# yaokeepmoving/distributed_tensorflow

Measured on AMD Instinct MI355X. Metric: images/sec (whole node) ResNet-50 bf16 at 1/2/4/8 MI355X; scaling efficiency, higher is better.
Workload: dtype bf16; 1 GPU; model=ResNet-50 v1.5, image_size=224, hiprio=True, hipgraph=True, graph_streams=2, global_batch=1024, per_gpu_batch=1024, parallelism=dp1, optimizer=SGD, allreduce_dtype=f32, zero1=False, forced_collective=False

## Files before the change

csrc/kernels/c3wgrad.hip:

```cpp
#include "gemm_core.h"

namespace dtf {
namespace {

constexpr int C3_SLOT = 72 * 128;
constexpr int C3_NS = 8;
constexpr int C3_DY = 64 * 128;
constexpr int C3_NB = 4;
constexpr int C3_JUNK = 8192;
constexpr int C3_SMEM = C3_NS * C3_SLOT + C3_NB * C3_DY + C3_JUNK;
constexpr int C3_OUT = 64 * 9 * 64;

struct C3Args {
  const bf16_t* X;
  const bf16_t* dY;
  float* ws;
  int H, W;
  long rows;
  int rpb;
};

__device__ __forceinline__ v8bf c3_tr_pair(uint32_t a0, uint32_t a1) {
  v4s r0, r1;
  asm volatile("ds_read_b64_tr_b16 %0, %1" : "=v"(r0) : "v"(a0));
// ... 92 lines not shown
  for (int it = 0; it < n_mine; ++it) {
    if (it + 2 < n_mine) asm volatile("s_waitcnt vmcnt(16)" ::: "memory");
    else if (it + 1 < n_mine) asm volatile("s_waitcnt vmcnt(8)" ::: "memory");
    else asm volatile("s_waitcnt vmcnt(0)" ::: "memory");
    asm volatile("s_waitcnt lgkmcnt(0)\n\ts_barrier" ::: "memory");
    if (it + C3_NB - 1 < n_mine) issue(it + C3_NB - 1, in, ih);
    next(in, ih);
    const char* img = dyi + (it % C3_NB) * C3_DY;
    const char* xr[3];
#pragma unroll
    for (int ta = 0; ta < 3; ++ta) xr[ta] = xs + ((n * VH + h + ta) & (C3_NS - 1)) * C3_SLOT;
    v8bf fx[2][9], fy[2][4];
    auto load = [&](int ks, v8bf(&x)[9], v8bf(&y)[4]) {
#pragma unroll
      for (int ta = 0; ta < 3; ++ta)
#pragma unroll
        for (int tb = 0; tb < 3; ++tb) x[ta * 3 + tb] = c3_frag(xr[ta], 16 * wave, tb, ks, lane);
#pragma unroll
      for (int j = 0; j < 4; ++j) y[j] = c3_frag(img, 16 * j, 0, ks, lane);
    };
    load(0, fx[0], fy[0]);
#pragma unroll
    for (int ks = 0; ks < 2; ++ks) {
      asm volatile("s_waitcnt lgkmcnt(0)" ::: "memory");
#pragma unroll
      for (int u = 0; u < 9; ++u) asm volatile("" : "+v"(fx[ks][u]));
#pragma unroll
      for (int j = 0; j < 4; ++j) asm volatile("" : "+v"(fy[ks][j]));
      if (ks == 0) load(1, fx[1], fy[1]);
#pragma unroll
      for (int u = 0; u < 9; ++u)
#pragma unroll
        for (int j = 0; j < 4; ++j)
          acc[u][j] = __builtin_amdgcn_mfma_f32_16x16x32_bf16(fx[ks][u], fy[ks][j], acc[u][j], 0, 0, 0);
    }
    next(n, h);
  }

  float* slab = a.ws + (long)blockIdx.x * C3_OUT;
#pragma unroll
  for (int u = 0; u < 9; ++u)
#pragma unroll
    for (int j = 0; j < 4; ++j) {
      const int k = 16 * j + (lane & 15), c = 16 * wave + 4 * (lane >> 4);
      *reinterpret_cast<float4*>(slab + ((long)k * 9 + u) * 64 + c) =
          make_float4(acc[u][j][0], acc[u][j][1], acc[u][j][2], acc[u][j][3]);
    }
}

}

int c3_wgrad_try(const void* X, const void* dY, float* dW, int N, int H, int W, int accumulate, float* ws,
                 long ws_elems, hipStream_t st) {
  if (((uintptr_t)X & 15) || ((uintptr_t)dY & 15) || !ws || N < 1 || H < 1 || W < 1 || W > 64) return -1;
  if ((long)N * (H + 2) >= (1l << 31)) return -1;
  C3Args a{};
  a.X = (const bf16_t*)X; a.dY = (const bf16_t*)dY; a.ws = ws;
  a.H = H; a.W = W;
  a.rows = (long)N * H;
  int grid = 256;
  while (grid > 8 && (long)grid * C3_OUT > ws_elems) grid /= 2;
  if ((long)grid * C3_OUT > ws_elems) return -1;
  a.rpb = (int)((a.rows + grid - 1) / grid);
  grid = (int)((a.rows + a.rpb - 1) / a.rpb);
  hipLaunchKernelGGL(c3_wgrad_kernel, dim3(grid), dim3(256), 0, st, a);
  if (hipGetLastError() != hipSuccess) return -1;
  dtf_sum_rows(ws, C3_OUT, grid, C3_OUT, dW, accumulate, st);
  return (int)hipGetLastError();
}

}
```

csrc/kernels/gemm.hip:

```cpp
#include <cstdlib>

#include "gemm_core.h"

__global__ void __launch_bounds__(256) dtf_group_rows_kernel(float* __restrict__ rows, long stride, int nrows,
                                                             int sg, long W, float* __restrict__ out,
                                                             int accumulate) {
  const long i = (long)blockIdx.x * blockDim.x + threadIdx.x;
  if (i >= W) return;
  const int r0 = blockIdx.y * sg;
  const int r1 = min(nrows, r0 + sg);
  float a8[8] = {0, 0, 0, 0, 0, 0, 0, 0};
  int r = r0;
  for (; r + 8 <= r1; r += 8) {
#pragma unroll
    for (int u = 0; u < 8; ++u) a8[u] += rows[(long)(r + u) * stride + i];
  }
  for (; r < r1; ++r) a8[0] += rows[(long)r * stride + i];
  const float acc = ((a8[0] + a8[1]) + (a8[2] + a8[3])) + ((a8[4] + a8[5]) + (a8[6] + a8[7]));
  if (out) out[i] = accumulate ? out[i] + acc : acc;
  else rows[(long)r0 * stride + i] = acc;
}

__global__ void __launch_bounds__(256) dtf_group_rows4_kernel(float* __restrict__ rows, long stride, int nrows,
                                                              int sg, long W4, float* __restrict__ out,
// ... 598 lines not shown
    long t = i;
    const int kc = (int)(t % k8); t /= k8;
    const int jw = (int)(t % nkw); t /= nkw;
    const int j = (int)(t % nkh);
    const int c = (int)(t / nkh);
    const long so = (((long)c * R + rh + sh * j) * S + rw + sw * jw) * K + kc * 8;
    *reinterpret_cast<uint4*>(dst + i * 8) = *reinterpret_cast<const uint4*>(src + so);
  }
}

static int conv_dgrad_impl(const void* dY, const void* Wcrsk, void* dX, int N, int H, int W, int C, int K, int R,
                           int S, int P, int Q, int sh, int sw, int ph, int pw, int dh, int dw, int out_f32,
                           float beta, int tile, void* ws, long ws_bf16, const void* bnx, const void* bnmask,
                           const float* bnmean, float* bnpart, int* bnrows, const void* betamask,
                           const void* bsrc2, void* stream, const void* bnrx = nullptr, const void* bnrw = nullptr);

namespace dtf {
int pwconv_dgrad_try(const void* dY, const void* Wck, void* dX, float beta, const void* betamask, const void* bnx,
                     const void* bnmask, const float* bnmean, float* part, long M, int Kc, int N, const void* bsrc2,
                     int H, int W, hipStream_t st, const void* bnrx, const void* bnrw);
}
static int g_pw_dgrad = -1;
static bool pwdgrad_enabled() {
  if (g_pw_dgrad < 0) {
    const char* e = getenv("DTF_PW_DGRAD");
    g_pw_dgrad = !(e && e[0] == '0');
  }
  return g_pw_dgrad != 0;
}
DTF_API int dtf_set_pw_dgrad(int on) {
  g_pw_dgrad = on ? 1 : 0;
  return 0;
}
namespace dtf {
int pw_wgrad_try(const void* X, const void* dY, float* dW, long P, int C, int K, int accumulate, float* ws,
                 long ws_elems, hipStream_t st, bool split_out);
}
namespace dtf {
int c3_wgrad_try(const void* X, const void* dY, float* dW, int N, int H, int W, int accumulate, float* ws,
                 long ws_elems, hipStream_t st);
}
static int g_c3_wgrad = -1;
static bool c3wgrad_enabled() {
  if (g_c3_wgrad < 0) {
    const char* e = getenv("DTF_C3_WGRAD");
    g_c3_wgrad = !(e && e[0] == '0');
  }
  return g_c3_wgrad != 0;
}
DTF_API int dtf_set_c3_wgrad(int on) {
  g_c3_wgrad = on ? 1 : 0;
  return 0;
}
static int g_pw_wgrad = -1;
static bool pwwgrad_enabled() {
  if (g_pw_wgrad < 0) {
    const char* e = getenv("DTF_PW_WGRAD");
    g_pw_wgrad = e ? atoi(e) : 1;
  }
  return g_pw_wgrad != 0;
}
DTF_API int dtf_set_pw_wgrad(int on) {
  g_pw_wgrad = on;
  return 0;
}

DTF_API int dtf_conv_dgrad(const void* dY, const void* Wcrsk, void* dX, int N, int H, int W, int C, int K, int R,
                           int S, int P, int Q, int sh, int sw, int ph, int pw, int dh, int dw, int out_f32,
                           float beta, int tile, void* ws, long ws_bf16, const void* bnx, const void* bnmask,
                           const float* bnmean, float* bnpart, int* bnrows, const void* betamask,
                           void* stream) {
  return conv_dgrad_impl(dY, Wcrsk, dX, N, H, W, C, K, R, S, P, Q, sh, sw, ph, pw, dh, dw, out_f32, beta, tile, ws,
                         ws_bf16, bnx, bnmask, bnmean, bnpart, bnrows, betamask, nullptr, stream);
}

DTF_API int dtf_conv_dgrad_x(const void* dY, const void* Wcrsk, void* dX, int N, int H, int W, int C, int K, int R,
                             int S, int P, int Q, int sh, int sw, int ph, int pw, int dh, int dw, float beta, void* ws,
                             long ws_bf16, const void* bnx, const void* bnmask, const float* bnmean, float* bnpart,
                             int* bnrows, const void* betamask, const void* bsrc2, const void* bnrx, const void* bnrw,
                             void* stream) {
  if (bsrc2) {
    if ((H & 1) || (W & 1) || R != 1 || S != 1 || sh != 1 || sw != 1 || ph != 0 || pw != 0) return -11;
    return conv_dgrad_impl(dY, Wcrsk, dX, N, H, W, C, K, 1, 1, H, W, 1, 1, 0, 0, 1, 1, 0, 1.f, -1, ws, ws_bf16, bnx,
                           bnmask, bnmean, bnpart, bnrows, nullptr, bsrc2, stream, bnrx, bnrw);
  }
  return conv_dgrad_impl(dY, Wcrsk, dX, N, H, W, C, K, R, S, P, Q, sh, sw, ph, pw, dh, dw, 0, beta, -1, ws, ws_bf16,
                         bnx, bnmask, bnmean, bnpart, bnrows, betamask, nullptr, stream, bnrx, bnrw);
}

DTF_API int dtf_conv_dgrad_addsub2(const void* dY, const void* Wcrsk, void* dX, const void* bsrc2, int N, int H, int W,
                                   int C, int K, int tile, void* ws, long ws_bf16, const void* bnx,
                                   const void* bnmask, const float* bnmean, float* bnpart, int* bnrows,
                                   void* stream) {
  if ((H & 1) || (W & 1) || !bsrc2) return -11;
  return conv_dgrad_impl(dY, Wcrsk, dX, N, H, W, C, K, 1, 1, H, W, 1, 1, 0, 0, 1, 1, 0, 1.f, tile, ws, ws_bf16, bnx,
                         bnmask, bnmean, bnpart, bnrows, nullptr, bsrc2, stream);
}

static int conv_dgrad_impl(const void* dY, const void* Wcrsk, void* dX, int N, int H, int W, int C, int K, int R,
                           int S, int P, int Q, int sh, int sw, int ph, int pw, int dh, int dw, int out_f32,
                           float beta, int tile, void* ws, long ws_bf16, const void* bnx, const void* bnmask,
                           const float* bnmean, float* bnpart, int* bnrows, const void* betamask,
                           const void* bsrc2, void* stream, const void* bnrx, const void* bnrw) {
  if ((C & 3) || (K & 7)) return -1;
  if (bnrx && (bnx || !bnrw || !bnpart || !bnmean || !bnrows)) return -9;
  if (bnx && (out_f32 || (C & 7) || !bnpart || !bnmean || !bnrows)) return -9;
// ... 84 lines not shown
      a.lda = K; a.ldb = (long)nkh * nkw * K; a.ldc = C;
      a.batch = 1; a.splitk = 1; a.kchunk = (a.K + BK - 1) / BK * BK;
      a.alpha = 1.f; a.beta = beta; a.act = 0; a.out_f32 = out_f32;
      a.crm = 1;
      a.dRm1 = make_fastdiv((uint32_t)(Hs * Ws)); a.dRm2 = make_fastdiv((uint32_t)Ws);
      a.rmH = H; a.rmW = W; a.rmsh = sh; a.rmsw = sw; a.rmh0 = h0; a.rmw0 = w0;
      bn_args(a);
      const bool pointwise = nkh == 1 && nkw == 1 && ch == 0 && cw == 0 && Hs == P && Ws == Q;
      const int am = pointwise ? OP_KCONTIG
                     : tap_uniform(K, nkh * nkw, (long)N * P * Q * K) ? OP_DGRAD_T : OP_DGRAD;
      int t = tile;
      if (t >= 0 && try_conv256(a, am, OP_KCONTIG, t, st)) {
      } else {
        dispatch(a, am, OP_KCONTIG, t < 0 ? pick_glds_tile(a, am, OP_KCONTIG) : t, st);
      }
      prow += a.tiles_m;
    }
  }
  if (bnrows) *bnrows = bnx ? prow : 0;
  return (int)hipGetLastError();
}

DTF_API int dtf_conv_wgrad(const void* X, const void* dY, float* dW, int N, int H, int W, int C, int K, int R,
                           int S, int P, int Q, int sh, int sw, int ph, int pw, int dh, int dw, int accumulate,
                           int splitk, int tile, float* ws, long ws_elems, void* stream) {
  if ((C & 7) || (K & 7)) return -1;
  const int splitk_req = splitk;
  if (tile < 0 && C == 16 && R == 4 && S == 4 && K == 64) tile = 3;
  hipStream_t st = (hipStream_t)stream;
  GemmArgs a{};
  a.g = make_geom(N, H, W, C, K, R, S, P, Q, sh, sw, ph, pw, dh, dw);
  a.g_rowrep = rowrep(a.g.R, a.g.S);
  a.A = (const bf16_t*)dY; a.B = (const bf16_t*)X;
  a.M = K; a.N = R * S * C; a.K = N * P * Q;
  a.lda = K; a.ldb = C; a.ldc = (long)R * S * C;
  a.batch = 1;
  a.alpha = 1.f; a.beta = 0.f; a.act = 0; a.out_f32 = 1;
  const long mn = (long)a.M * a.N;
  if (splitk <= 0) splitk = choose_splitk(a.M, a.N, a.K, 128, 128, 1);
  if (ws == nullptr || ws_elems < mn * 2) splitk = 1;
  else if ((long)splitk * mn > ws_elems) splitk = (int)(ws_elems / mn);
  if (splitk < 1) splitk = 1;
  a.splitk = splitk;
  a.kchunk = ((a.K + splitk - 1) / splitk + BK - 1) / BK * BK;
  bool pointwise = R == 1 && S == 1 && sh == 1 && sw == 1 && ph == 0 && pw == 0;
  if (pointwise && tile < 0 && splitk_req <= 0 && pwwgrad_enabled() &&
      pw_wgrad_try(X, dY, dW, (long)N * H * W, C, K, accumulate, ws, ws_elems, st, g_pw_wgrad == 2) == 0)
    return 0;
  if (tile < 0 && splitk_req <= 0 && C == 64 && K == 64 && R == 3 && S == 3 && sh == 1 && sw == 1 && ph == 1 &&
      pw == 1 && dh == 1 && dw == 1 && P == H && Q == W && c3wgrad_enabled() &&
      c3_wgrad_try(X, dY, dW, N, H, W, accumulate, ws, ws_elems, st) == 0)
    return 0;
  const bool small = (long)N * H * W * C * 2 < (1l << 31) && (long)N * P * Q * K * 2 < (1l << 31);
  const bool use_glds = small && (tile >= 7 || (tile < 0 && R * S > 1));
  const bool rowmap = small && (use_glds || !pointwise);
  constexpr bool swap_on = true;
  constexpr bool c256w = false;
  const bool c256_forced = tile >= 11 && tile <= 14;
  if (small && ws != nullptr && (c256_forced || (tile < 0 && c256w && conv256_on())) &&
      (pointwise || (C % 8 == 0 && (dh == 1 && dw == 1)))) {
    GemmArgs b = a;
    b.A = (const bf16_t*)X; b.B = (const bf16_t*)dY;
    b.M = R * S * C; b.N = K;
    b.lda = C; b.ldb = K; b.ldc = K;
    const int cfg = c256_forced ? tile - 11 : (K <= 64 ? 2 : K >= 256 ? 1 : 0);
    const int bn = cfg == 1 ? 256 : cfg == 2 ? 64 : 128;
    const long mnT = (long)b.M * b.N;
    const long tiles = (long)cdiv(b.M, 256) * cdiv(b.N, bn);
    long sk = std::max<long>(1, (512 + tiles - 1) / tiles);
    sk = std::min<long>(sk, std::max<long>(1, (long)b.K / 1024));
    if ((sk + 1) * mnT > ws_elems) sk = ws_elems / mnT - 1;
    if (sk >= 1) {
      b.splitk = (int)sk;
      b.kchunk = (int)(((b.K + sk - 1) / sk + BK - 1) / BK * BK);
      b.C = ws;
      b.slab = mnT;
      b.beta = 0.f;
      b.atomic_out = 0;
      if (conv256_try(b, pointwise ? OP_KOUTER : OP_WGRADX_R, OP_KOUTER_R, cfg, st, true) == 0) {
        float* dwt = ws + (long)b.splitk * mnT;
        dtf_sum_rows(ws, mnT, b.splitk, mnT, dwt, 0, st);
        hipLaunchKernelGGL(transpose_acc_kernel, dim3(cdiv(b.N, 32), cdiv(b.M, 32)), dim3(256), 0, st, dwt, dW,
                           b.M, b.N, accumulate);
        return (int)hipGetLastError();
      }
    }
  }
  if (c256_forced) tile = -1;
  if (pointwise && tile < 0 && ws != nullptr && K >= 128 && C >= 128 && (long)K * C >= 4 * 256 * 128) {
    int bn = 0;
    const int s = plan_w4_split_long(a.M, a.N, a.K, 1, bn);
    if (bn && s >= 1 && (s == 1 || (long)s * mn <= ws_elems)) {
      GemmArgs b = a;
      b.splitk = s;
      b.kchunk = ((b.K + s - 1) / s + BK - 1) / BK * BK;
      if (s > 1) {
        b.C = ws;
        b.slab = mn;
        b.beta = 0.f;
      } else {
        b.C = dW;
        b.beta = accumulate ? 1.f : 0.f;
      }
      if (tile256_try(b, OP_KOUTER, OP_KOUTER, st, bn) == 0) {
        if (s > 1) {
          count_launch(LC_SPLITK);
          dtf_sum_rows(ws, mn, s, mn, dW, accumulate, st);
        }
        return (int)hipGetLastError();
      }
    }
  }
  if (swap_on && use_glds && tile < 0 && K <= 64 && R * S > 1 && ws != nullptr) {
    GemmArgs b = a;
    b.A = (const bf16_t*)X; b.B = (const bf16_t*)dY;
    b.M = R * S * C; b.N = K;
    b.lda = C; b.ldb = K; b.ldc = K;
    const long mnT = (long)b.M * b.N;
    int sk = choose_splitk(b.M, b.N, b.K, 128, 64, 1);
    if ((long)(sk + 1) * mnT > ws_elems) sk = (int)(ws_elems / mnT) - 1;
    if (sk >= 1) {
      b.splitk = sk;
      b.kchunk = ((b.K + sk - 1) / sk + BK - 1) / BK * BK;
      b.C = ws;
      b.slab = mnT;
      b.beta = 0.f;
      dispatch(b, OP_WGRADX_R, OP_KOUTER_R, 8, st);
      float* dwt = ws + (long)sk * mnT;
      dtf_sum_rows(ws, mnT, sk, mnT, dwt, 0, st);
      hipLaunchKernelGGL(transpose_acc_kernel, dim3(cdiv(b.N, 32), cdiv(b.M, 32)), dim3(256), 0, st, dwt, dW, b.M,
                         b.N, accumulate);
      return (int)hipGetLastError();
    }
  }
  if (tile < 0 && use_glds) tile = 7;
  if (tile < 0) {
    if (a.M <= 64) tile = pointwise && a.N >= 256 ? 4 : 3;
    else if (R * S > 1) tile = 0;
  }
  auto run = [&]() {
    dispatch(a, rowmap ? OP_KOUTER_R : OP_KOUTER, rowmap ? OP_WGRADX_R : pointwise ? OP_KOUTER : OP_WGRADX, tile, st);
  };
  if (splitk == 1) {
    a.C = dW;
    a.beta = accumulate ? 1.f : 0.f;
    run();
    return (int)hipGetLastError();
  }
  a.C = ws;
  a.slab = mn;
  run();
  dtf_sum_rows(ws, mn, splitk, mn, dW, accumulate, st);
  return (int)hipGetLastError();
}
```

csrc/kernels/gemm_core.h:

```cpp
#pragma once
#include "common.h"
#include <algorithm>
#include <type_traits>

namespace dtf {

enum OpMode : int {
  OP_KCONTIG = 0,
  OP_KOUTER = 1,
  OP_IM2COL = 2,
  OP_DGRAD = 3,
  OP_WGRADX = 4,
  OP_IM2COL_T = 5,
  OP_DGRAD_T = 6,
  OP_KOUTER_R = 7,
  OP_WGRADX_R = 8,
};

struct ConvGeom {
  int N, H, W, C;
  int Kout, R, S;
  int P, Q;
  int sh, sw, ph, pw, dh, dw;
  FastDiv dPQ, dQ, dHW, dW, dC, dS, dK;
};

struct GemmArgs {
  const bf16_t* A;
  const bf16_t* B;
  void* C;
  bf16_t* aux;
  const float* bias;
  const float* scales;
  float* stats;
  long lda, ldb, ldc;
  long sA, sB, sC;
  int M, N, K;
  int batch, splitk, kchunk;
  int tiles_m, tiles_n;
  float alpha, beta;
  int act;
  int out_f32;
  int atomic_out;
  long slab;
  ConvGeom g;
  uint64_t g_rowrep;
  const bf16_t* bnx;
  const uint8_t* bnmask;
  const float* bnmean;
  const uint8_t* betamask;
  const bf16_t* dact_src;
  int dact;
  float* zero_slot;
  const bf16_t* bsrc;
  FastDiv dBhw, dBw;
  int bH2, bW2;
  int crm;
  FastDiv dRm1, dRm2;
  int rmH, rmW, rmsh, rmsw, rmh0, rmw0;
  uint8_t* q8;
  uint8_t* q8T;
  float* q8col;
  const float* q8scale;
  float* q8amax;
  const float* q8amax_prev;
  float* q8used;
  float* q8used2;
  int q8fmt;
  int no_c;
  int aux_nt;
  float* rowsum;
};

__device__ __forceinline__ uint32_t q8pack4(int fmt, float a0, float a1, float a2, float a3) {
  int r;
  if (fmt) {
    r = __builtin_amdgcn_cvt_pk_bf8_f32(a0, a1, 0, false);
    r = __builtin_amdgcn_cvt_pk_bf8_f32(a2, a3, r, true);
  } else {
    r = __builtin_amdgcn_cvt_pk_fp8_f32(a0, a1, 0, false);
    r = __builtin_amdgcn_cvt_pk_fp8_f32(a2, a3, r, true);
  }
  return (uint32_t)r;
}

__device__ __forceinline__ long out_row(const GemmArgs& a, int m) {
  if (!a.crm) return m;
  uint32_t n, hw, hh, ww;
  fdivmod((uint32_t)m, a.dRm1, n, hw);
  fdivmod(hw, a.dRm2, hh, ww);
  return ((long)n * a.rmH + (long)(a.rmsh * (int)hh + a.rmh0)) * a.rmW + (a.rmsw * (int)ww + a.rmw0);
}

constexpr int BK = 64;
constexpr int NT = 256;

__device__ __forceinline__ const bf16_t* beta_src(const GemmArgs& a, long m, int n, const bf16_t* cp) {
  if (!a.bsrc) return cp;
  uint32_t nn, hw, h, w;
  fdivmod((uint32_t)m, a.dBhw, nn, hw);
  fdivmod(hw, a.dBw, h, w);
  if ((h | w) & 1u) return nullptr;
  return a.bsrc + (((long)nn * a.bH2 + (h >> 1)) * a.bW2 + (w >> 1)) * a.ldc + n;
}

__device__ __forceinline__ void stat_acc(const GemmArgs& a, long mrow, int n, const float (&v)[4], float (&cs)[4],
                                         float (&cq)[4]) {
  if (a.bnx) {
    const long e = mrow * a.ldc + n;
    const uint2 xr = *reinterpret_cast<const uint2*>(a.bnx + e);
    const float x[4] = {__uint_as_float(xr.x << 16), __uint_as_float(xr.x & 0xffff0000u),
                        __uint_as_float(xr.y << 16), __uint_as_float(xr.y & 0xffff0000u)};
    const uint32_t bits = a.bnmask ? ((uint32_t)a.bnmask[e >> 3] >> (e & 4)) : 0xFu;
    const float4 mu = *reinterpret_cast<const float4*>(a.bnmean + n);
    const float m4[4] = {mu.x, mu.y, mu.z, mu.w};
#pragma unroll
    for (int r = 0; r < 4; ++r) {
      const float dz = ((bits >> r) & 1u) ? v[r] : 0.f;
      cs[r] += dz;
      cq[r] = fmaf(dz, x[r] - m4[r], cq[r]);
    }
  } else {
#pragma unroll
    for (int r = 0; r < 4; ++r) { cs[r] += v[r]; cq[r] = fmaf(v[r], v[r], cq[r]); }
// ... 976 lines not shown
```

csrc/kernels/gemm_w4.h:

```cpp
#pragma once
#include <type_traits>

#include "gemm_core.h"

namespace dtf {
namespace {

constexpr int W4_THREADS = 256;
constexpr int W4_A = 256 * BK * 2;

__device__ __forceinline__ void w4_barrier() {
  __builtin_amdgcn_sched_barrier(0);
  asm volatile("" ::: "memory");
  __builtin_amdgcn_s_barrier();
  asm volatile("" ::: "memory");
  __builtin_amdgcn_sched_barrier(0);
}

__device__ __forceinline__ void w4_mfma_drain() {
  asm volatile("s_nop 7\n\ts_nop 7\n\ts_nop 7" ::: "memory");
}

__device__ __forceinline__ void w4_lgkm0() {
  __builtin_amdgcn_sched_barrier(0);
// ... 64 lines not shown
    dS = g.dS;
    if constexpr (MODE == OP_IM2COL_T) {
      dCh = g.dC;
      tsh = g.dh * g.W * g.C * 2;
      tsw = g.dw * g.C * 2;
      rsrc = __builtin_amdgcn_make_buffer_rsrc((void*)p, (short)0, (int)((long)g.N * g.H * g.W * g.C * 2), 0x00020000);
    } else {
      dCh = g.dK;
      tsh = -(g.dh * g.Q * g.Kout * 2);
      tsw = -(g.dw * g.Kout * 2);
      rsrc = __builtin_amdgcn_make_buffer_rsrc((void*)p, (short)0, (int)((long)g.N * g.P * g.Q * g.Kout * 2),
                                               0x00020000);
    }
#pragma unroll
    for (int i = 0; i < L; ++i) {
      const int row = 32 * i + (t >> 3);
      const int c = (t & 7) ^ ((row >> 1) & 7);
      const int r = r0 + row;
      uint32_t m = 0u;
      int off = 0;
      if (r < Rtot) {
        uint32_t n, rem, y, x;
        if constexpr (MODE == OP_IM2COL_T) {
          fdivmod((uint32_t)r, g.dPQ, n, rem);
          fdivmod(rem, g.dQ, y, x);
          const int hb = (int)y * g.sh - g.ph, wb = (int)x * g.sw - g.pw;
          off = (((int)n * g.H + hb) * g.W + wb) * g.C * 2;
          m = tap_mask(g.R, g.S, max(0, -hb), min(g.R - 1, g.H - 1 - hb), max(0, -wb), min(g.S - 1, g.W - 1 - wb),
                       a.g_rowrep);
        } else {
          fdivmod((uint32_t)r, g.dHW, n, rem);
          fdivmod(rem, g.dW, y, x);
          const int hb = (int)y + g.ph, wb = (int)x + g.pw;
          off = (((int)n * g.P + hb) * g.Q + wb) * g.Kout * 2;
          m = tap_mask(g.R, g.S, max(0, hb - g.P + 1), min(g.R - 1, hb), max(0, wb - g.Q + 1), min(g.S - 1, wb),
                       a.g_rowrep);
        }
      }
      roff[i] = off + c * 16;
      tmask[i] = m;
    }
  }
  __device__ __forceinline__ void issue1(int k0, uint32_t lds, int i) {
    uint32_t tap, c0, kh, kw;
    fdivmod((uint32_t)k0, dCh, tap, c0);
    fdivmod(tap, dS, kh, kw);
    const int toff = (int)kh * tsh + (int)kw * tsw + (int)c0 * 2;
    const uint32_t off = ((tmask[i] >> tap) & 1u) ? (uint32_t)(roff[i] + toff) : 0x80000000u;
    __builtin_amdgcn_raw_ptr_buffer_load_lds(rsrc, (__attribute__((address_space(3))) void*)(uintptr_t)(lds + i * 4096),
                                             16, off, 0, 0, 0);
  }
};

template <int R, int MODE>
using W4LoaderFor = typename std::conditional<MODE == OP_IM2COL_T || MODE == OP_DGRAD_T, W4Gather<R, MODE>,
                                              W4Loader<R, MODE>>::type;

}
}
```

csrc/kernels/gemm_w4.hip:

```cpp
#include <cstdlib>

#include "gemm_w4.h"

namespace dtf {
namespace {


template <int BN>
struct W4Geo {
  static constexpr int JN = BN / 32;
  static constexpr int B_BYTES = BN * BK * 2;
  static constexpr int STAGE = W4_A + B_BYTES;
  static constexpr int EPI = 256 * (BN + 8) * 2;
  static constexpr int SMEM = EPI > 2 * STAGE ? EPI : 2 * STAGE;
  static constexpr int SMEM_ST = EPI + 16384 > 2 * STAGE ? EPI + 16384 : 2 * STAGE;
  static constexpr int NSTEP = 2 * JN;
  static constexpr int NREAD = 8 + JN;
  static constexpr int NG = 8 + BN / 32;
};

__device__ __forceinline__ void w4_mfma(v4f& c, const v8bf& b, const v8bf& a) {
  asm volatile("v_mfma_f32_16x16x32_bf16 %0, %1, %2, %0" : "+a"(c) : "v"(b), "v"(a));
}
template <int R>
__device__ __forceinline__ v8bf w4_frag_kouter(const char* lds, int cb, int kk, int lane) {
  const int G = lane >> 4, i = lane & 15, q = i >> 2, p = i & 3;
  v4s r[2];
#pragma unroll
  for (int h = 0; h < 2; ++h) {
    const int k = 32 * kk + 8 * G + 4 * h + q;
    const int g = ((cb >> 2) + p) ^ (kouter_swz<R>(k) << 2);
    const uint32_t addr = (uint32_t)(uintptr_t)LDS_PTR(char, lds + k * (R * 2) + g * 8);
    asm volatile("ds_read_b64_tr_b16 %0, %1" : "=v"(r[h]) : "v"(addr));
  }
  v8s both = __builtin_shufflevector(r[0], r[1], 0, 1, 2, 3, 4, 5, 6, 7);
  return __builtin_bit_cast(v8bf, both);
}
template <int R, int MODE>
__device__ __forceinline__ v8bf w4_frag(const char* lds, int rb, int kk, int lane) {
  if constexpr (MODE == OP_KOUTER) return w4_frag_kouter<R>(lds, rb, kk, lane);
  else return frag_kcontig(lds, rb, kk, lane);
}
template <int BN, bool ST = false>
__device__ __forceinline__ void w4_epilogue(const GemmArgs& a, v4f (&acc)[8][BN / 32], char* smem, int m0, int n0,
                                            int z, int bz) {
  constexpr int JN = BN / 32, WTN = BN / 2;
  const int lane = threadIdx.x & 63, wave = threadIdx.x >> 6;
  const int wm = wave >> 1, wn = wave & 1;
  const long cbase = a.slab > 0 ? (long)z * a.slab : (long)bz * a.sC;
  const float alpha = a.alpha;
  if (a.out_f32) {
    float* C = reinterpret_cast<float*>(a.C) + cbase;
#pragma unroll
    for (int i = 0; i < 8; ++i) {
      const int m = m0 + wm * 128 + i * 16 + (lane & 15);
      if (m >= a.M) continue;
      float* crow = C + (long)m * a.ldc;
#pragma unroll
      for (int j = 0; j < JN; ++j) {
        const int n = n0 + wn * WTN + j * 16 + (lane >> 4) * 4;
        if (n >= a.N) continue;
        float4 v = make_float4(alpha * acc[i][j][0], alpha * acc[i][j][1], alpha * acc[i][j][2], alpha * acc[i][j][3]);
        if (a.beta != 0.f) {
          const float4 o = *reinterpret_cast<const float4*>(crow + n);
          v.x += a.beta * o.x; v.y += a.beta * o.y; v.z += a.beta * o.z; v.w += a.beta * o.w;
        }
        *reinterpret_cast<float4*>(crow + n) = v;
      }
    }
    return;
  }
  constexpr int CS = BN + 8;
  bf16_t* ct = reinterpret_cast<bf16_t*>(smem);
  float csum[ST ? JN : 1][4], csq[ST ? JN : 1][4];
  if constexpr (ST) {
#pragma unroll
    for (int j = 0; j < JN; ++j)
#pragma unroll
      for (int r = 0; r < 4; ++r) csum[j][r] = csq[j][r] = 0.f;
  }
  float4 bias[JN];
#pragma unroll
  for (int j = 0; j < JN; ++j) {
    const int n = n0 + wn * WTN + j * 16 + (lane >> 4) * 4;
    bias[j] = (a.bias && n < a.N) ? *reinterpret_cast<const float4*>(a.bias + n) : make_float4(0.f, 0.f, 0.f, 0.f);
  }
#pragma unroll
  for (int i = 0; i < 8; ++i) {
    const int ml = wm * 128 + i * 16 + (lane & 15);
    const int m = m0 + ml;
#pragma unroll
    for (int j = 0; j < JN; ++j) {
      const int nl = wn * WTN + j * 16 + (lane >> 4) * 4;
// ... 123 lines not shown
  }
#pragma unroll 4
  for (int it = 0; it < 256 / RPP; ++it) {
    const int ml = r0 + RPP * it;
    const int m = m0 + ml;
    if (m >= a.M) break;
    uint4 val = *reinterpret_cast<const uint4*>(ct + ml * CS + c8 * 8);
    const long e = (long)m * a.ldc + n;
    if (a.beta != 0.f) {
      const uint4 old = *reinterpret_cast<const uint4*>(C + e);
      const uint32_t vw[4] = {val.x, val.y, val.z, val.w}, ow[4] = {old.x, old.y, old.z, old.w};
      uint32_t rw[4];
#pragma unroll
      for (int q = 0; q < 4; ++q) {
        const float f0 = __uint_as_float(vw[q] << 16) + a.beta * __uint_as_float(ow[q] << 16);
        const float f1 = __uint_as_float(vw[q] & 0xffff0000u) + a.beta * __uint_as_float(ow[q] & 0xffff0000u);
        rw[q] = pack2bf(f0, f1);
      }
      val = make_uint4(rw[0], rw[1], rw[2], rw[3]);
    }
    if (a.dact) val = dact8(val, *reinterpret_cast<const uint4*>(a.dact_src + e), a.dact);
    *reinterpret_cast<uint4*>(C + e) = val;
  }
}

template <int AM, int BMODE, int BN, int VAR = 0>
__global__ void __launch_bounds__(W4_THREADS, 1) gemm_w4_kernel(GemmArgs a) {
  using G = W4Geo<BN>;
  constexpr int JN = G::JN, WTN = BN / 2, NSTEP = G::NSTEP, NREAD = G::NREAD, NG = G::NG;
  constexpr int SPR = JN / 4;
  constexpr bool ST = (VAR & 16) != 0;
  __shared__ __attribute__((aligned(16))) char smem[ST ? G::SMEM_ST : G::SMEM];
  const int lane = threadIdx.x & 63, wave = threadIdx.x >> 6;
  const int wm = wave >> 1, wn = wave & 1;

  const int nwg = a.tiles_m * a.tiles_n;
  int bid, z;
  xcd_block(nwg, bid, z);
  constexpr int GROUP = 4;
  const int per_group = GROUP * a.tiles_n;
  const int grp = bid / per_group;
  const int first_m = grp * GROUP;
  const int gsize = min(a.tiles_m - first_m, GROUP);
  const int in_g = bid - grp * per_group;
  const int tile_m = first_m + in_g % gsize;
  const int tile_n = in_g / gsize;
  const int m0 = tile_m * 256, n0 = tile_n * BN;
  const int bz = z / a.splitk, sk = z % a.splitk;
  const int kbeg = sk * a.kchunk;
  const int kend = min(a.K, kbeg + a.kchunk);
  const int nk = kend > kbeg ? (kend - kbeg + BK - 1) / BK : 0;

  W4LoaderFor<256, AM> la;
  W4Loader<BN, BMODE> lb;
  la.init(a, a.A + (long)bz * a.sA, a.lda, m0, a.M, threadIdx.x);
  lb.init(a, a.B + (long)bz * a.sB, a.ldb, n0, a.N, threadIdx.x);
  const uint32_t lds0 = (uint32_t)(uintptr_t)(__attribute__((address_space(3))) char*)smem +
                        (uint32_t)__builtin_amdgcn_readfirstlane(wave) * 1024u;

  v4f acc[8][JN];
#pragma unroll
  for (int i = 0; i < 8; ++i)
#pragma unroll
    for (int j = 0; j < JN; ++j) acc[i][j] = (v4f){0.f, 0.f, 0.f, 0.f};
  v8bf fa0[8], fb0[JN], fa1[8], fb1[JN];
  constexpr bool RS = (VAR & 8) != 0;
  float rs[8];
#pragma unroll
  for (int i = 0; i < 8; ++i) rs[i] = 0.f;

  auto issue1 = [&](int t, int s) {
    const uint32_t st = lds0 + (uint32_t)((t & 1) * G::STAGE);
    const int k0 = kbeg + min(t, nk - 1) * BK;
    if (s < 8) la.issue1(k0, st, s);
    else lb.issue1(k0, st + W4_A, s - 8);
  };
  auto issue = [&](int t) {
#pragma unroll
    for (int s = 0; s < NG; ++s) issue1(t, s);
  };
  auto read1 = [&](v8bf (&fa)[8], v8bf (&fb)[JN], int t, int kk, int s) {
    const char* st = smem + (t & 1) * G::STAGE;
    if (s < JN) fb[s] = w4_frag<BN, BMODE>(st + W4_A, wn * WTN + s * 16, kk, lane);
    else fa[s - JN] = w4_frag<256, AM>(st, wm * 128 + (s - JN) * 16, kk, lane);
  };
  auto read = [&](v8bf (&fa)[8], v8bf (&fb)[JN], int t, int kk) {
#pragma unroll
    for (int s = 0; s < NREAD; ++s) read1(fa, fb, t, kk, s);
  };
  auto mma4 = [&](const v8bf (&fa)[8], const v8bf (&fb)[JN], int s) {
    const int i = s / SPR, j0 = (s % SPR) * 4;
#pragma unroll
    for (int j = 0; j < 4; ++j) w4_mfma(acc[i][j0 + j], fb[j0 + j], fa[i]);
    if constexpr (RS) {
      if (s % SPR == 0) {
        typedef __bf16 bf2_t __attribute__((ext_vector_type(2)));
        const bf2_t one = {(__bf16)1.0f, (__bf16)1.0f};
        const v8bf f = fa[i];
        float r = rs[i];
        r = __builtin_amdgcn_fdot2_f32_bf16(__builtin_shufflevector(f, f, 0, 1), one, r, false);
        r = __builtin_amdgcn_fdot2_f32_bf16(__builtin_shufflevector(f, f, 2, 3), one, r, false);
        r = __builtin_amdgcn_fdot2_f32_bf16(__builtin_shufflevector(f, f, 4, 5), one, r, false);
        r = __builtin_amdgcn_fdot2_f32_bf16(__builtin_shufflevector(f, f, 6, 7), one, r, false);
        rs[i] = r;
      }
    }
  };
  auto reads_at = [&](v8bf (&fa)[8], v8bf (&fb)[JN], int t, int kk, int s) {
    constexpr int H = NSTEP / 2;
    if (s < H) {
#pragma unroll
      for (int r = s * NREAD / H; r < (s + 1) * NREAD / H; ++r) read1(fa, fb, t, kk, r);
    }
  };

  if (nk > 0) issue(0);
  if (nk > 1) {
    issue(1);
    if constexpr (NG == 16) asm volatile("s_waitcnt vmcnt(16)" ::: "memory");
    else asm volatile("s_waitcnt vmcnt(12)" ::: "memory");
  } else {
    asm volatile("s_waitcnt vmcnt(0)" ::: "memory");
  }
  w4_barrier();
  if (nk > 0) {
    read(fa0, fb0, 0, 0);
    if constexpr ((VAR & 2) != 0) read(fa1, fb1, 0, 1);
  }

  for (int t = 0; t + 1 < nk; ++t) {
    w4_lgkm0();
#pragma unroll
    for (int s = 0; s < NSTEP; ++s) {
      if constexpr (!(VAR & 2)) reads_at(fa1, fb1, t, 1, s);
      mma4(fa0, fb0, s);
      __builtin_amdgcn_sched_barrier(0);
    }
    asm volatile("s_waitcnt vmcnt(0) lgkmcnt(0)" ::: "memory");
    w4_barrier();
#pragma unroll
    for (int s = 0; s < NSTEP; ++s) {
      if constexpr (!(VAR & 1)) {
#pragma unroll
        for (int g = s * NG / NSTEP; g < (s + 1) * NG / NSTEP; ++g) issue1(t + 2, g);
      }
      if constexpr (!(VAR & 2)) reads_at(fa0, fb0, t + 1, 0, s);
      mma4(fa1, fb1, s);
      __builtin_amdgcn_sched_barrier(0);
    }
  }
  if (nk > 0) {
    w4_lgkm0();
#pragma unroll
    for (int s = 0; s < NSTEP; ++s) {
      reads_at(fa1, fb1, nk - 1, 1, s);
      mma4(fa0, fb0, s);
      __builtin_amdgcn_sched_barrier(0);
    }
    w4_lgkm0();
#pragma unroll
    for (int s = 0; s < NSTEP; ++s) mma4(fa1, fb1, s);
  }
  w4_mfma_drain();
  if constexpr (RS) {
    if (tile_n == 0 && wn == 0 && a.rowsum) {
#pragma unroll
      for (int i = 0; i < 8; ++i) {
        float v = rs[i];
        v += __shfl_xor(v, 16, 64);
        v += __shfl_xor(v, 32, 64);
        const int m = m0 + wm * 128 + i * 16 + lane;
        if (lane < 16 && m < a.M) a.rowsum[(long)z * a.M + m] = v;
      }
    }
  }
  asm volatile("s_waitcnt vmcnt(0)" ::: "memory");
  __syncthreads();
  if constexpr ((VAR & 4) != 0) {
    float x = 0.f;
#pragma unroll
    for (int i = 0; i < 8; ++i)
#pragma unroll
      for (int j = 0; j < JN; ++j) x += acc[i][j][0] + acc[i][j][3];
    if (x == 12345.f) reinterpret_cast<float*>(a.C)[threadIdx.x] = x;
    return;
  }
  w4_epilogue<BN, ST>(a, acc, smem, m0, n0, z, bz);
}

template <int AM, int BMODE, int BN, int VAR>
void w4_go(GemmArgs& a, hipStream_t st) {
  dim3 grid(a.tiles_m * a.tiles_n, 1, a.batch * a.splitk);
  hipLaunchKernelGGL((gemm_w4_kernel<AM, BMODE, BN, VAR>), grid, dim3(W4_THREADS), 0, st, a);
}

template <int BN, int VAR = 0>
void w4_launch(GemmArgs& a, int amode, int bmode, hipStream_t st) {
  a.tiles_m = cdiv(a.M, 256);
  a.tiles_n = cdiv(a.N, BN);
  if constexpr (VAR != 0) {
    w4_go<OP_KCONTIG, OP_KCONTIG, BN, VAR>(a, st);
    return;
  }
  if (a.rowsum) {
    w4_go<OP_KOUTER, OP_KOUTER, BN, 8>(a, st);
    return;
  }
  if (amode == OP_IM2COL_T) {
    if (a.stats) w4_go<OP_IM2COL_T, OP_KCONTIG, BN, 16>(a, st);
    else w4_go<OP_IM2COL_T, OP_KCONTIG, BN, 0>(a, st);
    return;
  }
  if (amode == OP_DGRAD_T) {
    if (a.stats) w4_go<OP_DGRAD_T, OP_KCONTIG, BN, 16>(a, st);
    else w4_go<OP_DGRAD_T, OP_KCONTIG, BN, 0>(a, st);
    return;
  }

  if (amode == OP_KCONTIG && bmode == OP_KCONTIG) w4_go<OP_KCONTIG, OP_KCONTIG, BN, VAR>(a, st);
  else if (amode == OP_KCONTIG) w4_go<OP_KCONTIG, OP_KOUTER, BN, VAR>(a, st);
  else if (bmode == OP_KCONTIG) w4_go<OP_KOUTER, OP_KCONTIG, BN, VAR>(a, st);
  else w4_go<OP_KOUTER, OP_KOUTER, BN, VAR>(a, st);
}

}

bool gemm_w4_ok(const GemmArgs& a, int amode, int bmode) {
  if (a.atomic_out || a.crm || a.bsrc || a.betamask || a.scales || a.q8 || a.q8T || a.q8col || a.zero_slot)
    return false;
  if (a.stats && ((amode != OP_IM2COL_T && amode != OP_DGRAD_T) || (amode == OP_DGRAD_T) != (a.bnx != nullptr) ||
                  a.out_f32 || a.beta != 0.f || a.bias || a.act || a.aux || a.dact || a.batch > 1 || a.splitk > 1 ||
                  (a.bnx && (a.N & 7))))
    return false;
  if (a.bnx && !a.stats) return false;
  if (amode == OP_IM2COL_T || amode == OP_DGRAD_T) {
    const ConvGeom& g = a.g;
    const bool fwd = amode == OP_IM2COL_T;
    if (bmode != OP_KCONTIG || ((fwd ? g.C : g.Kout) & 63) || g.R * g.S > 32 ||
        (fwd ? (long)g.N * g.H * g.W * g.C : (long)g.N * g.P * g.Q * g.Kout) * 2 >= (1l << 31) ||
        (!fwd && (g.sh != 1 || g.sw != 1)) ||
        a.batch > 1 || a.splitk > 1 || a.out_f32 || (a.N & 7) || (a.ldc & 7) || ((uintptr_t)a.C & 15) ||
        (a.K % BK) || (a.ldb & 7) || ((uintptr_t)a.A & 15) || ((uintptr_t)a.B & 15) ||
        (long)a.N * a.ldb * 2 >= (1l << 31))
      return false;
    return true;
  }
  if (a.out_f32 ? (a.bias || a.act || a.aux || a.dact || (a.ldc & 3) || ((uintptr_t)a.C & 15))
                : ((a.N & 7) || (a.ldc & 7) || ((uintptr_t)a.C & 15)))
    return false;
  if ((amode != OP_KCONTIG && amode != OP_KOUTER) || (bmode != OP_KCONTIG && bmode != OP_KOUTER)) return false;
  if (a.rowsum && (!a.out_f32 || amode != OP_KOUTER || bmode != OP_KOUTER || a.batch > 1)) return false;
  if (a.kchunk % BK || a.K % BK || (a.lda & 7) || (a.ldb & 7)) return false;
  if (((uintptr_t)a.A & 15) || ((uintptr_t)a.B & 15)) return false;
  auto fits = [](long elems) { return elems * 2 < (1l << 31); };
  if (amode == OP_KCONTIG ? !fits((long)a.M * a.lda) : (!fits((long)a.K * a.lda) || (a.M & 7))) return false;
  if (bmode == OP_KCONTIG ? !fits((long)a.N * a.ldb) : (!fits((long)a.K * a.ldb) || (a.N & 7))) return false;
  return true;
}

int gemm_w4_try(GemmArgs& a, int amode, int bmode, hipStream_t st, int bn) {
  if (!gemm_w4_ok(a, amode, bmode)) return 1;
  count_launch(bn == 128 ? LC_W4_128 : LC_W4_256);
  if (bn == 128) w4_launch<128>(a, amode, bmode, st);
  else w4_launch<256>(a, amode, bmode, st);
  return 0;
}

}

DTF_API int dtf_gemm_w4_var(const void* A, const void* B, void* C, int M, int N, int K, int var, int bn,
                            void* stream) {
  using namespace dtf;
  GemmArgs a{};
  a.A = (const bf16_t*)A; a.B = (const bf16_t*)B; a.C = C;
  a.M = M; a.N = N; a.K = K; a.lda = K; a.ldb = K; a.ldc = N;
  a.batch = 1; a.splitk = 1; a.kchunk = K; a.alpha = 1.f;
  if ((N & 7) || (K % BK) || (bn != 128 && bn != 256)) return -1;
  hipStream_t st = (hipStream_t)stream;
  const int m = OP_KCONTIG;
  if (bn == 128) {
    if (var == 1) w4_launch<128, 1>(a, m, m, st);
    else if (var == 2) w4_launch<128, 2>(a, m, m, st);
    else if (var == 3) w4_launch<128, 3>(a, m, m, st);
    else if (var == 4) w4_launch<128, 4>(a, m, m, st);
    else w4_launch<128, 0>(a, m, m, st);
  } else {
    if (var == 1) w4_launch<256, 1>(a, m, m, st);
    else if (var == 2) w4_launch<256, 2>(a, m, m, st);
    else if (var == 3) w4_launch<256, 3>(a, m, m, st);
    else if (var == 4) w4_launch<256, 4>(a, m, m, st);
    else w4_launch<256, 0>(a, m, m, st);
  }
  return (int)hipGetLastError();
}

DTF_API int dtf_gemm_w4(const void* A, const void* B, void* C, int M, int N, int K, long lda, long ldb, long ldc,
                        int a_kouter, int b_kouter, int out_f32, int bn, void* stream) {
  dtf::GemmArgs a{};
  a.A = (const bf16_t*)A; a.B = (const bf16_t*)B; a.C = C;
  a.M = M; a.N = N; a.K = K; a.lda = lda; a.ldb = ldb; a.ldc = ldc;
  a.batch = 1; a.splitk = 1; a.kchunk = K; a.alpha = 1.f; a.beta = 0.f; a.out_f32 = out_f32;
  if ((N & 3) || (K % dtf::BK)) return -1;
  if (dtf::gemm_w4_try(a, a_kouter ? dtf::OP_KOUTER : dtf::OP_KCONTIG, b_kouter ? dtf::OP_KOUTER : dtf::OP_KCONTIG,
                       (hipStream_t)stream, bn))
    return -2;
  return (int)hipGetLastError();
}
```

distributed_tensorflow_amd/_native.py:

```python
from __future__ import annotations

import ctypes
import os
import threading

_LIBDIR = os.path.join(os.path.dirname(os.path.abspath(__file__)), "lib")
_lock = threading.Lock()
_kern = None
_rt = None

P, I, L, F, U = ctypes.c_void_p, ctypes.c_int, ctypes.c_long, ctypes.c_float, ctypes.c_ulonglong

_KERNEL_SIGS = {
    "dtf_stream_create": [I],
    "dtf_gemm": [P, P, P, P, P, P, P, I, I, I, L, L, L, I, I, I, L, L, L, F, F, I, I, I, I, P, L, P],
    "dtf_conv_fwd": [P, P, P, P, P, P] + [I] * 15 + [I, I, I, P],
    "dtf_pwconv_fwd": [P, P, P, P, P, L, I, I, P],
    "dtf_conv_bn_apply_fwd": [P, P, P, P, P, P, P, P, L, I, I, I, P, P, P, P, P, F, F, P, P, P, P, P],
    "dtf_conv_dgrad": [P, P, P] + [I] * 15 + [I, F, I, P, L, P, P, P, P, P, P, P],
    "dtf_conv_dgrad_addsub2": [P, P, P, P, I, I, I, I, I, I, P, L, P, P, P, P, P, P],
    "dtf_conv_fwd_bn": [P, P, P, P] + [I] * 15 + [I, P, P, P, P, F, F, P, P, P, P, P, P],
    "dtf_conv_dgrad_x": [P, P, P] + [I] * 15 + [F, P, L, P, P, P, P, P, P, P, P, P, P],
    "dtf_bn_bwd_apply_coef": [P, P, P, L, I, P, P, P, P, P, P, P, P],
    "dtf_set_ew_variant": [I],
    "dtf_set_pw_dgrad": [I],
    "dtf_pw_conv_bwd": [P, P, P, P, P, I, P, P, P, P, P, P, L, L, I, I, P],
    "dtf_pw_conv_bwd_bn": [P, P, P, P, P, P, P, P, I, P, P, P, P, P, P, L, L, I, I, P, P, P, P, P, P],
    "dtf_bn_bwd_coef": [P, I, P, P, P, L, I, P, P, I, P, P],
    "dtf_set_pw_wgrad": [I],
    "dtf_set_c3_wgrad": [I],
    "dtf_set_split_penalty": [I],
    "dtf_set_ew_apply_nu": [I],
    "dtf_bn_bwd_partials": [P, P, P, P, P, P, L, I, P, P, P, P, I, P, I, P, P, P, P, P, P],
    "dtf_conv_wgrad": [P, P, P] + [I] * 15 + [I, I, I, P, L, P],
    "dtf_stem_wgrad": [P, P, P, I, I, I, I, P, L, P],
    "dtf_stem_wgrad_fused": [P, P, P, P, P, P, I, I, I, I, P, L, P],
    "dtf_bn_stats": [P, L, I, P, P, P],
    "dtf_bn_finalize": [P, I, P, P, P, P, L, I, F, F, P, P, P, P, P],
    "dtf_bn_infer_coeff": [P, P, P, P, I, F, P, P, P],
    "dtf_bn_apply": [P, P, P, P, P, L, I, I, P, P, P, P],
    "dtf_bn_bwd": [P, P, P, P, P, P, P, L, I, P, P, P, P, I, P, P, P, P, P, P],
    "dtf_layernorm_fwd": [P, P, P, P, P, P, L, I, F, P],
    "dtf_layernorm_bwd": [P, P, P, P, P, P, P, P, L, L, I, I, P],
    "dtf_layernorm_bwd2": [P, P, P, P, P, P, P, P, L, L, I, I, P, P],
    "dtf_add_dropout_layernorm_fwd": [P, P, P, P, P, P, P, P, L, I, F, F, U, P, P],
    "dtf_layernorm_bwd_part": [P, P, P, P, P, P, P, L, L, I, P, P, P, F, U, P, P],
    "dtf_maxpool_fwd": [P, P, P] + [I] * 12 + [P],
    "dtf_maxpool_bwd": [P, P, P] + [I] * 12 + [P],
    "dtf_add_dropout": [P, P, P, L, F, U, P, P],
    "dtf_softmax_ce_fwd": [P, I, P, P, P, L, I, F, P],
    "dtf_softmax_ce_bwd": [P, I, P, P, P, P, L, I, F, P],
    "dtf_nchw_to_s2d": [P, P, I, I, I, I, P],
    "dtf_stem_fwd": [P, P, P, P, P] + [I] * 9 + [P],
    "dtf_bn_relu_maxpool_fwd": [P, P, P, P, P] + [I] * 12 + [P],
    "dtf_maxpool_bn_bwd": [P, P, P, P, P, P] + [I] * 12 + [P, P, P, I, P, P],
    "dtf_gap_fwd": [P, P, I, I, I, I, P],
    "dtf_gap_bwd": [P, I, P, I, I, I, P],
    "dtf_optim_apply": [I, P, P, P, P, P, L, F, F, F, F, F, F, F, I, I, P, P, P, P],
    "dtf_sumsq": [P, L, P, I, P],
    "dtf_hp_ring_select": [P, I, I, P, P, P],
    "dtf_lw_tile_elems": [],
    "dtf_lw_pass1": [I, P, P, I, I, L, L, P, P, P, P, P, P, F, F, F, F, F, F, P, P, P, P],
    "dtf_lw_finalize": [I, I, P, P, I, I, L, L, P, P, P, P, F, F, F, P, P],
    "dtf_lw_pass2": [I, P, P, I, I, L, L, P, P, P, P, P, P, F, F, I, I, P, P, P, P],
    "dtf_cast_f32_bf16": [P, P, L, P],
    "dtf_cast_bf16_f32": [P, P, L, P],
    "dtf_nchw_to_nhwc_pad": [P, P, I, I, I, I, P],
    "dtf_filter_to_crsk": [P, P, I, I, I, P],
    "dtf_filters_to_crsk": [P, I, I, P],
    "dtf_add_bf16": [P, P, P, L, F, F, P],
    "dtf_act": [P, P, P, L, I, I, P],
    "dtf_dropout": [P, P, L, F, U, P, P],
    "dtf_rng_advance": [P, P],
    "dtf_gemm256": [P, P, P, I, I, I, L, L, L, I, I, I, I, P, L, P],
    "dtf_gemm_w4": [P, P, P, I, I, I, L, L, L, I, I, I, I, P],
    "dtf_gemm_w4_var": [P, P, P, I, I, I, I, I, P],
    "dtf_gemm_w4_fp8": [P, P, P, I, I, I, L, L, L, I, I, I, P],
    "dtf_fp8_w4_enable": [I],
    "dtf_gemm_wgrad_bias": [P, P, P, P, I, I, I, L, L, L, F, P, L, P],
    "dtf_launch_counts": [P, I],
    "dtf_xs_epoch_inc": [P, I, P],
    "dtf_xs_signal": [P, I, P, I, P],
    "dtf_xs_wait": [P, I, P, I, P, I, P],
# ... 107 lines not shown
```

Measured before the change: 15530 images/sec.

## Route 3x3 conv weight-gradient through w4 GEMM with pixel-table gather loader

Adds a new B-operand loader mode for the w4 GEMM kernel that gathers im2col input patches for spatial (R*S>1) weight gradients. It uses a precomputed per-output-pixel table of base offsets plus row/column validity bits, built by a small extra kernel. Default-enabled conv wgrad dispatch now tries this path for C>=128, K>=256 shapes before falling back to the older glds implicit-GEMM path. The aim is to reuse the optimized w4 pipeline for 3x3/7x7-free shapes, at the cost of an extra table kernel launch and workspace use. It also tightens the c3 specialist kernel to require H>=3.

```diff
diff --git a/csrc/kernels/c3wgrad.hip b/csrc/kernels/c3wgrad.hip
--- a/csrc/kernels/c3wgrad.hip
+++ b/csrc/kernels/c3wgrad.hip
@@ -168,7 +168,7 @@
 
 int c3_wgrad_try(const void* X, const void* dY, float* dW, int N, int H, int W, int accumulate, float* ws,
                  long ws_elems, hipStream_t st) {
-  if (((uintptr_t)X & 15) || ((uintptr_t)dY & 15) || !ws || N < 1 || H < 1 || W < 1 || W > 64) return -1;
+  if (((uintptr_t)X & 15) || ((uintptr_t)dY & 15) || !ws || N < 1 || H < 3 || W < 1 || W > 64) return -1;
   if ((long)N * (H + 2) >= (1l << 31)) return -1;
   C3Args a{};
   a.X = (const bf16_t*)X; a.dY = (const bf16_t*)dY; a.ws = ws;
diff --git a/csrc/kernels/gemm.hip b/csrc/kernels/gemm.hip
--- a/csrc/kernels/gemm.hip
+++ b/csrc/kernels/gemm.hip
@@ -674,6 +674,48 @@
   g_c3_wgrad = on ? 1 : 0;
   return 0;
 }
+static int g_w4_wgrad3 = -1;
+static bool w4wgrad3_enabled() {
+  if (g_w4_wgrad3 < 0) {
+    const char* e = getenv("DTF_W4_WGRAD3");
+    g_w4_wgrad3 = !(e && e[0] == '0');
+  }
+  return g_w4_wgrad3 != 0;
+}
+DTF_API int dtf_set_w4_wgrad3(int on) {
+  g_w4_wgrad3 = on ? 1 : 0;
+  return 0;
+}
+
+static int w4_wgrad3_try(const GemmArgs& g, float* dW, int accumulate, float* ws, long ws_elems, hipStream_t st,
+                         int bn, int s) {
+  if (g.M < 256) return 1;
+  GemmArgs b = g;
+  if (bn <= 0) bn = 256;
+  if (s <= 0) s = g.splitk;
+  if (bn != 128 && bn != 256) return 1;
+  const long mn = (long)b.M * b.N;
+  const long slabs = s > 1 ? (long)s * mn : 0;
+  if (!ws || slabs + b.K > ws_elems) return 1;
+  b.pixtab = reinterpret_cast<uint32_t*>(ws + slabs);
+  if (s > 1) {
+    b.C = ws;
+    b.slab = mn;
+    b.beta = 0.f;
+  } else {
+    b.C = dW;
+    b.beta = accumulate ? 1.f : 0.f;
+  }
+  b.splitk = s;
+  b.kchunk = ((b.K + s - 1) / s + BK - 1) / BK * BK;
+  if (gemm_w4_try(b, OP_KOUTER, OP_WGRADX_R, st, bn)) return 1;
+  if (s > 1) {
+    count_launch(LC_SPLITK);
+    dtf_sum_rows(ws, mn, s, mn, dW, accumulate, st);
+  }
+  return 0;
+}
+
 static int g_pw_wgrad = -1;
 static bool pwwgrad_enabled() {
   if (g_pw_wgrad < 0) {
@@ -864,6 +906,9 @@
       c3_wgrad_try(X, dY, dW, N, H, W, accumulate, ws, ws_elems, st) == 0)
     return 0;
   const bool small = (long)N * H * W * C * 2 < (1l << 31) && (long)N * P * Q * K * 2 < (1l << 31);
+  if (tile < 0 && splitk_req <= 0 && R * S > 1 && dh == 1 && dw == 1 && small && C >= 128 && K >= 256 &&
+      a.kchunk >= 128 * BK && w4wgrad3_enabled() && w4_wgrad3_try(a, dW, accumulate, ws, ws_elems, st, 0, 0) == 0)
+    return (int)hipGetLastError();
   const bool use_glds = small && (tile >= 7 || (tile < 0 && R * S > 1));
   const bool rowmap = small && (use_glds || !pointwise);
   constexpr bool swap_on = true;
@@ -965,3 +1010,26 @@
   dtf_sum_rows(ws, mn, splitk, mn, dW, accumulate, st);
   return (int)hipGetLastError();
 }
+
+DTF_API int dtf_conv_wgrad3_w4(const void* X, const void* dY, float* dW, int N, int H, int W, int C, int K, int R,
+                               int S, int P, int Q, int sh, int sw, int ph, int pw, int accumulate, int splitk,
+                               int bn, float* ws, long ws_elems, void* stream) {
+  if ((C & 7) || (K & 7) || K < 256 || (long)N * H * W * C * 2 >= (1l << 31) ||
+      (long)N * P * Q * K * 2 >= (1l << 31))
+    return -2;
+  GemmArgs a{};
+  a.g = make_geom(N, H, W, C, K, R, S, P, Q, sh, sw, ph, pw, 1, 1);
+  a.g_rowrep = rowrep(a.g.R, a.g.S);
+  a.A = (const bf16_t*)dY; a.B = (const bf16_t*)X;
+  a.M = K; a.N = R * S * C; a.K = N * P * Q;
+  a.lda = K; a.ldb = C; a.ldc = (long)R * S * C;
+  a.batch = 1;
+  a.alpha = 1.f; a.out_f32 = 1;
+  a.splitk = choose_splitk(a.M, a.N, a.K, 128, 128, 1);
+  const long mn = (long)a.M * a.N;
+  if (ws == nullptr || ws_elems < mn * 2) a.splitk = 1;
+  else if ((long)a.splitk * mn > ws_elems) a.splitk = (int)(ws_elems / mn);
+  if (a.splitk < 1) a.splitk = 1;
+  if (w4_wgrad3_try(a, dW, accumulate, ws, ws_elems, (hipStream_t)stream, bn, splitk)) return -2;
+  return (int)hipGetLastError();
+}
diff --git a/csrc/kernels/gemm_core.h b/csrc/kernels/gemm_core.h
--- a/csrc/kernels/gemm_core.h
+++ b/csrc/kernels/gemm_core.h
@@ -70,6 +70,7 @@
   int no_c;
   int aux_nt;
   float* rowsum;
+  uint32_t* pixtab;
 };
 
 __device__ __forceinline__ uint32_t q8pack4(int fmt, float a0, float a1, float a2, float a3) {
diff --git a/csrc/kernels/gemm_w4.h b/csrc/kernels/gemm_w4.h
--- a/csrc/kernels/gemm_w4.h
+++ b/csrc/kernels/gemm_w4.h
@@ -140,9 +140,56 @@
   }
 };
 
+constexpr int W4_PT_ROW = 24, W4_PT_COL = 27;
+constexpr uint32_t W4_PT_NEVER = 0x80000000u;
+
+template <int R>
+struct W4GatherK {
+  static constexpr int L = R / 32;
+  static constexpr int KS = 64 / L;
+  __amdgpu_buffer_rsrc_t rsrc, trsrc;
+  int coff[L];
+  uint32_t need[L];
+  uint32_t ent[L];
+  int kr4;
+  int C2;
+
+  __device__ __forceinline__ void init(const GemmArgs& a, const bf16_t* p, long, int r0, int Rtot, int t) {
+    const ConvGeom& g = a.g;
+    C2 = g.C * 2;
+    rsrc = __builtin_amdgcn_make_buffer_rsrc((void*)p, (short)0, (int)((long)g.N * g.H * g.W * g.C * 2), 0x00020000);
+    trsrc = __builtin_amdgcn_make_buffer_rsrc((void*)a.pixtab, (short)0, (int)((long)a.K * 4), 0x00020000);
+    const int kr0 = t / (R / 8);
+    kr4 = kr0 * 4;
+#pragma unroll
+    for (int i = 0; i < L; ++i) {
+      const int kr = kr0 + i * KS;
+      const int c = (t % (R / 8)) ^ (kouter_swz<R>(kr) << 1);
+      const int col = r0 + c * 8;
+      uint32_t tap, ci, kh, kw;
+      fdivmod((uint32_t)(col < Rtot ? col : 0), g.dC, tap, ci);
+      fdivmod(tap, g.dS, kh, kw);
+      need[i] = col < Rtot ? (1u << (W4_PT_ROW + kh)) | (1u << (W4_PT_COL + kw)) : W4_PT_NEVER;
+      coff[i] = (((int)kh * g.dh - g.ph) * g.W + (int)kw * g.dw - g.pw) * g.C * 2 + (int)ci * 2;
+    }
+  }
+  __device__ __forceinline__ void prefetch(int k0, int i) {
+    ent[i] = __builtin_amdgcn_raw_buffer_load_b32(trsrc, kr4 + i * KS * 4, k0 * 4, 0);
+  }
+  __device__ __forceinline__ void issue1(int, uint32_t lds, int i) {
+    const uint32_t e = ent[i];
+    uint32_t in = __umul24(e, (uint32_t)C2) + (uint32_t)coff[i];
+    asm volatile("" : "+v"(in));
+    const uint32_t off = (e & need[i]) == need[i] ? in : 0x80000000u;
+    __builtin_amdgcn_raw_ptr_buffer_load_lds(rsrc, (__attribute__((address_space(3))) void*)(uintptr_t)(lds + i * 4096),
+                                             16, off, 0, 0, 0);
+  }
+};
+
 template <int R, int MODE>
-using W4LoaderFor = typename std::conditional<MODE == OP_IM2COL_T || MODE == OP_DGRAD_T, W4Gather<R, MODE>,
-                                              W4Loader<R, MODE>>::type;
+using W4LoaderFor = typename std::conditional<
+    MODE == OP_IM2COL_T || MODE == OP_DGRAD_T, W4Gather<R, MODE>,
+    typename std::conditional<MODE == OP_WGRADX_R, W4GatherK<R>, W4Loader<R, MODE>>::type>::type;
 
 }
 }
diff --git a/csrc/kernels/gemm_w4.hip b/csrc/kernels/gemm_w4.hip
--- a/csrc/kernels/gemm_w4.hip
+++ b/csrc/kernels/gemm_w4.hip
@@ -38,7 +38,7 @@
 }
 template <int R, int MODE>
 __device__ __forceinline__ v8bf w4_frag(const char* lds, int rb, int kk, int lane) {
-  if constexpr (MODE == OP_KOUTER) return w4_frag_kouter<R>(lds, rb, kk, lane);
+  if constexpr (MODE == OP_KOUTER || MODE == OP_WGRADX_R) return w4_frag_kouter<R>(lds, rb, kk, lane);
   else return frag_kcontig(lds, rb, kk, lane);
 }
 template <int BN, bool ST = false>
@@ -268,7 +268,7 @@
   const int nk = kend > kbeg ? (kend - kbeg + BK - 1) / BK : 0;
 
   W4LoaderFor<256, AM> la;
-  W4Loader<BN, BMODE> lb;
+  W4LoaderFor<BN, BMODE> lb;
   la.init(a, a.A + (long)bz * a.sA, a.lda, m0, a.M, threadIdx.x);
   lb.init(a, a.B + (long)bz * a.sB, a.ldb, n0, a.N, threadIdx.x);
   const uint32_t lds0 = (uint32_t)(uintptr_t)(__attribute__((address_space(3))) char*)smem +
@@ -290,6 +290,9 @@
     const int k0 = kbeg + min(t, nk - 1) * BK;
     if (s < 8) la.issue1(k0, st, s);
     else lb.issue1(k0, st + W4_A, s - 8);
+    if constexpr (BMODE == OP_WGRADX_R) {
+      if (s >= 8) lb.prefetch(kbeg + min(t + 1, nk - 1) * BK, s - 8);
+    }
   };
   auto issue = [&](int t) {
 #pragma unroll
@@ -330,6 +333,11 @@
     }
   };
 
+  if (nk > 0) {
+#pragma unroll
+    for (int i = 0; i < BN / 32; ++i)
+      if constexpr (BMODE == OP_WGRADX_R) lb.prefetch(kbeg, i);
+  }
   if (nk > 0) issue(0);
   if (nk > 1) {
     issue(1);
@@ -404,6 +412,21 @@
   w4_epilogue<BN, ST>(a, acc, smem, m0, n0, z, bz);
 }
 
+__global__ void __launch_bounds__(256) w4_pixtab_kernel(uint32_t* __restrict__ tab, int npix, ConvGeom g) {
+  const int k = blockIdx.x * 256 + threadIdx.x;
+  if (k >= npix) return;
+  uint32_t n, pq, p, q;
+  fdivmod((uint32_t)k, g.dPQ, n, pq);
+  fdivmod(pq, g.dQ, p, q);
+  const int hb = (int)p * g.sh, wb = (int)q * g.sw;
+  uint32_t e = (uint32_t)(((int)n * g.H + hb) * g.W + wb);
+  for (int kh = 0; kh < g.R; ++kh)
+    if ((uint32_t)(hb - g.ph + kh * g.dh) < (uint32_t)g.H) e |= 1u << (W4_PT_ROW + kh);
+  for (int kw = 0; kw < g.S; ++kw)
+    if ((uint32_t)(wb - g.pw + kw * g.dw) < (uint32_t)g.W) e |= 1u << (W4_PT_COL + kw);
+  tab[k] = e;
+}
+
 template <int AM, int BMODE, int BN, int VAR>
 void w4_go(GemmArgs& a, hipStream_t st) {
   dim3 grid(a.tiles_m * a.tiles_n, 1, a.batch * a.splitk);
@@ -430,6 +453,10 @@
   if (amode == OP_DGRAD_T) {
     if (a.stats) w4_go<OP_DGRAD_T, OP_KCONTIG, BN, 16>(a, st);
     else w4_go<OP_DGRAD_T, OP_KCONTIG, BN, 0>(a, st);
+    return;
+  }
+  if (bmode == OP_WGRADX_R) {
+    w4_go<OP_KOUTER, OP_WGRADX_R, BN, 0>(a, st);
     return;
   }
 
@@ -461,6 +488,20 @@
       return false;
     return true;
   }
+  if (amode == OP_WGRADX_R) return false;
+  if (bmode == OP_WGRADX_R) {
+    const ConvGeom& g = a.g;
+    if (amode != OP_KOUTER) return false;
+    if (!a.out_f32 || a.bias || a.act || a.aux || a.dact || a.stats || a.rowsum || a.batch > 1) return false;
+    if ((g.C & 7) || (g.Kout & 7) || (a.K % BK) || (a.kchunk % BK) || (a.ldc & 3)) return false;
+    if (((uintptr_t)a.A & 15) || ((uintptr_t)a.B & 15) || ((uintptr_t)a.C & 15)) return false;
+    if ((long)g.N * g.H * g.W * g.C * 2 >= (1l << 31) || (long)a.K * g.Kout * 2 >= (1l << 31)) return false;
+    if (a.K != g.N * g.P * g.Q || a.lda != g.Kout) return false;
+    if (!a.pixtab || ((uintptr_t)a.pixtab & 3) || g.R > 3 || g.S > 3 || (long)g.N * g.H * g.W >= (1l << 24) ||
+        g.C * 2 >= (1 << 24) || (g.P - 1) * g.sh >= g.H || (g.Q - 1) * g.sw >= g.W)
+      return false;
+    return true;
+  }
   if (a.out_f32 ? (a.bias || a.act || a.aux || a.dact || (a.ldc & 3) || ((uintptr_t)a.C & 15))
                 : ((a.N & 7) || (a.ldc & 7) || ((uintptr_t)a.C & 15)))
     return false;
@@ -476,6 +517,8 @@
 
 int gemm_w4_try(GemmArgs& a, int amode, int bmode, hipStream_t st, int bn) {
   if (!gemm_w4_ok(a, amode, bmode)) return 1;
+  if (bmode == OP_WGRADX_R)
+    hipLaunchKernelGGL(w4_pixtab_kernel, dim3(cdiv(a.K, 256)), dim3(256), 0, st, a.pixtab, a.K, a.g);
   count_launch(bn == 128 ? LC_W4_128 : LC_W4_256);
   if (bn == 128) w4_launch<128>(a, amode, bmode, st);
   else w4_launch<256>(a, amode, bmode, st);
diff --git a/distributed_tensorflow_amd/_native.py b/distributed_tensorflow_amd/_native.py
--- a/distributed_tensorflow_amd/_native.py
+++ b/distributed_tensorflow_amd/_native.py
@@ -29,6 +29,8 @@
     "dtf_bn_bwd_coef": [P, I, P, P, P, L, I, P, P, I, P, P],
     "dtf_set_pw_wgrad": [I],
     "dtf_set_c3_wgrad": [I],
+    "dtf_set_w4_wgrad3": [I],
+    "dtf_conv_wgrad3_w4": [P, P, P] + [I] * 13 + [I, I, I, P, L, P],
     "dtf_set_split_penalty": [I],
     "dtf_set_ew_apply_nu": [I],
     "dtf_bn_bwd_partials": [P, P, P, P, P, P, L, I, P, P, P, P, I, P, I, P, P, P, P, P, P],
```

Result: faster. 15720 images/sec, median of 6 (+1.2%).
